# Liz490/multimodal_alzheimer

Hardware: AMD Instinct MI355X
Metric: volumes/sec fwd+bwd, 3D-ResNet-10 @128^3 bf16, 1/2/4/8 MI355X; % HBM roofline (higher is better)
Workload: dtype bf16; 1 GPU; BASELINE config 2: Anat_CNN ResNet-10 MRI-only, 1x128^3, batch 8/GPU, weighted CE, Adam, fwd+bwd+step; global_batch=8, parallelism=dp1, step_launch=hip graph replay

## Files before the change

### multimodal_alzheimer_amd/csrc/conv.hip

```cpp
#include <cstring>

#include "common.h"
#include "reduce.h"
#include "patchconv.h"
#include "pointwise.h"
#include "stem.h"

namespace {

constexpr int MAXTAPS = 344;
constexpr int TAPB = ((3 * MAXTAPS * 4 + 15) / 16) * 16;
constexpr int RB = 128;

struct Geom {
  int M, Nd, Cs, K, Kpad, cs_shift, taps, nb;
  int Ds, Hs, Ws, Dd, Hd, Wd;
  int KD, KH, KW;
  int sd, sh, sw, pd, ph, pw, dd, dh, dw;
  const void* res;
  int relu;
};

enum { FWD = 0, DGRAD = 1 };

// ... 1272 lines not shown
                                                          dst, stats, st);
      if (cfg == 5)
        return launch_igemm_bm<T, 256, MODE, 256, 2, 4, 4, 64>(g, m_max, classes, src, w, bias,
                                                              dst, stats, st);
      if (cfg == 6)
        return launch_igemm_bm<T, 256, MODE, 256, 2, 4, 3, 64>(g, m_max, classes, src, w, bias,
                                                              dst, stats, st);
    }
  }
  const bool small = igemm_bm(m_max * classes, g) == 64;
  if constexpr (sizeof(T) == 2) {
    if (igemm_nst(g, MODE) == 3) {
      if (bn_of(g) == 64)
        return small ? launch_igemm_bm<T, 64, MODE, 64, 2, 2, 3>(g, m_max, classes, src, w, bias, dst, stats, st)
                     : launch_igemm_bm<T, 64, MODE, 128, 2, 2, 3>(g, m_max, classes, src, w, bias, dst, stats, st);
      return small ? launch_igemm_bm<T, 128, MODE, 64, 2, 2, 3>(g, m_max, classes, src, w, bias, dst, stats, st)
                   : launch_igemm_bm<T, 128, MODE, 128, 2, 2, 3>(g, m_max, classes, src, w, bias, dst, stats, st);
    }
  }
  if (bn_of(g) == 64)
    return small ? launch_igemm_bm<T, 64, MODE, 64>(g, m_max, classes, src, w, bias, dst, stats, st)
                 : launch_igemm_bm<T, 64, MODE, 128>(g, m_max, classes, src, w, bias, dst, stats, st);
  return small ? launch_igemm_bm<T, 128, MODE, 64>(g, m_max, classes, src, w, bias, dst, stats, st)
               : launch_igemm_bm<T, 128, MODE, 128>(g, m_max, classes, src, w, bias, dst, stats, st);
}

template <int MODE>
int run_igemm(const Geom& g, int dtype, int64_t m_max, int classes, const void* src,
              const void* w, const float* bias, void* dst, float* stats, hipStream_t st) {
  if (dtype == MMAD_BF16)
    return run_igemm_t<u16, MODE>(g, m_max, classes, src, w, bias, dst, stats, st);
  return run_igemm_t<float, MODE>(g, m_max, classes, src, w, bias, dst, stats, st);
}

int wgrad_xcd() {
  static const int v = [] { const char* e = getenv("MMAD_WGRAD_XCD"); return e ? atoi(e) : 1; }();
  return v;
}

template <typename T, int BMW, int WBK, int NST, int WBNT, int WGM, int WGN, bool XFIX>
int launch_wgrad_x(const Geom& g, const WSplit& sp, const void* x, const void* dy, float* ws,
                   hipStream_t st) {
  const size_t lds = TAPB + NST * WBK * (BMW + WBNT) * sizeof(T);
  static const bool ok = set_lds(wgrad_kernel<T, BMW, WBK, NST, WBNT, WGM, WGN, XFIX>, lds);
  if (!ok) return MMAD_EUNSUPPORTED;
  const uint32_t xb = (uint32_t)((int64_t)g.nb * g.Ds * g.Hs * g.Ws * g.Cs * sizeof(T));
  const uint32_t yb = (uint32_t)((int64_t)g.M * g.Nd * sizeof(T));
  dim3 grid((unsigned)cdiv(g.K, WBNT), (unsigned)cdiv(g.Nd, BMW), (unsigned)sp.splits);
  hipLaunchKernelGGL((wgrad_kernel<T, BMW, WBK, NST, WBNT, WGM, WGN, XFIX>), grid,
                     dim3(64 * WGM * WGN), lds, st, g, (const T*)x, (const T*)dy, ws,
                     sp.m_per_split, xb, yb, wgrad_xcd());
  return launch_status();
}

template <typename T, int BMW, int WBK, int NST, int WBNT = WBN, int WGM = 2, int WGN = 2>
int launch_wgrad_k(const Geom& g, const WSplit& sp, const void* x, const void* dy, float* ws,
                   hipStream_t st) {
  if ((int64_t)g.nb * g.Ds * g.Hs * g.Ws * g.Cs * (int64_t)sizeof(T) >= (int64_t(1) << 31) ||
      (int64_t)g.M * g.Nd * (int64_t)sizeof(T) >= (int64_t(1) << 31))
    return MMAD_EUNSUPPORTED;
  if (WBK % g.Wd == 0)
    return launch_wgrad_x<T, BMW, WBK, NST, WBNT, WGM, WGN, true>(g, sp, x, dy, ws, st);
  return launch_wgrad_x<T, BMW, WBK, NST, WBNT, WGM, WGN, false>(g, sp, x, dy, ws, st);
}

int wgrad_1x1_nst() {
  static const int v = [] { const char* e = getenv("MMAD_WGRAD_1X1_NST"); return e ? atoi(e) : 3; }();
  return v;
}

template <typename T, int BMW>
int launch_wgrad(const Geom& g, const WSplit& sp, const void* x, const void* dy, float* ws,
                 hipStream_t st) {
  if (g.taps == 1 && wgrad_1x1_nst() == 3) return launch_wgrad_k<T, BMW, 32, 3>(g, sp, x, dy, ws, st);
  return launch_wgrad_k<T, BMW, 32, 2>(g, sp, x, dy, ws, st);
}

unsigned grid_for(int64_t total, int block = 256) {
  return (unsigned)std::max<int64_t>(1, std::min<int64_t>(cdiv(total, block), 65536));
}

enum Leaf { STEM, LATTICE5, LATTICE_ZP, LATTICE, LATTICE8, PATCHZ, PATCH, S2, PW, IGEMM, NONE };
enum Epi { EPI_NONE, EPI_RES, EPI_BNSUM };
bool leaf_has(Leaf l, Epi e) {
  if (e == EPI_RES) return l != STEM && l != PW;
  if (e == EPI_BNSUM) return l == LATTICE_ZP || l == LATTICE8 || l == PATCH;
  return true;
}
struct Route { Leaf leaf; int64_t tiles; };

Route resolve(const mmad_conv_desc* d, const Geom& g, int dtype, Epi epi, bool launch = true) {
  const Route none{NONE, -1};
  auto pick = [&](Leaf l, int64_t tiles) { return leaf_has(l, epi) ? Route{l, tiles} : none; };
  const bool u = d != nullptr && unfolded(d);
  if (u && epi != EPI_NONE) return none;
  if (u && mmad_stem::fwd_ok(d, dtype) && stem_kernel_on())
    return pick(STEM, mmad_stem::fwd_stats_rows(d));
  if (launch && !geom_ok(g, dtype)) return none;
  if (!u && dtype == MMAD_BF16) {
    const mmad_patch::Geo q = patch_geo(g);
    if (g.sd == 1 && g.sh == 1 && g.sw == 1) {
      if (mmad_lattice5::ok(q)) return pick(LATTICE5, mmad_lattice5::tiles(q));
      const bool zp = mmad_lattice_zp::ok(q);
      const int64_t lt = zp ? mmad_lattice_zp::tiles(q) : mmad_lattice::tiles(q);
      if (mmad_lattice::ok(q, lt)) return pick(zp ? LATTICE_ZP : LATTICE, lt);
      if (mmad_lattice8::ok(q)) return pick(LATTICE8, mmad_lattice8::tiles(q));
      if (mmad_patch::ok(q))
        return mmad_patchz::ok(q) ? pick(PATCHZ, mmad_patchz::tiles(q))
                                  : pick(PATCH, mmad_patch::tiles(q));
    }
    if (mmad_s2::ok(q, g.sd, g.sh, g.sw)) return pick(S2, mmad_s2::tiles(q));
  }
  if (d != nullptr && leaf_has(PW, epi) && mmad_pw::fwd_ok(d, dtype))
    return pick(PW, mmad_pw::fwd_tiles(d));
  return pick(IGEMM, cdiv(g.M, fwd_tile_rows(g, dtype)));
}

int launch_route(const Route& r, const mmad_conv_desc* d, const Geom& g, int dtype,
                 const mmad_patch::Geo& q, const void* x, const void* wp, const float* bias,
                 void* y, float* stats, void* stream) {
  switch (r.leaf) {
    case STEM: return mmad_stem::fwd(d, x, wp, bias, y, stats, stream);
    case LATTICE5: return mmad_lattice5::fwd(q, x, wp, bias, y, stats, stream);
    case LATTICE_ZP: return mmad_lattice_zp::fwd(q, x, wp, bias, y, stats, stream);
    case LATTICE: return mmad_lattice::fwd(q, x, wp, bias, y, stats, stream);
    case LATTICE8: return mmad_lattice8::fwd(q, x, wp, bias, y, stats, stream);
    case PATCHZ: return mmad_patchz::fwd(q, x, wp, bias, y, stats, stream);
    case PATCH: return mmad_patch::fwd(q, x, wp, bias, y, stats, stream);
    case S2: return mmad_s2::fwd(q, g.sd, g.sh, g.sw, x, wp, bias, y, stats, stream);
    case PW: return mmad_pw::fwd(d, x, wp, bias, y, stats, stream);
    case IGEMM: return run_igemm<FWD>(g, dtype, g.M, 1, x, wp, bias, y, stats, as_stream(stream));
    case NONE: break;
  }
  return MMAD_EUNSUPPORTED;
}

Route dgrad_fwd_route(const mmad_conv_desc* d, int dtype, Epi epi, Geom* gf) {
  if (!desc_ok(d) || (dtype != MMAD_F32 && dtype != MMAD_BF16) || unfolded(d) ||
      mmad_pw::ok(d, dtype) || !dgrad_as_fwd(d))
    return Route{NONE, -1};
  *gf = dgrad_fwd_geom(d, dtype);
  return resolve(nullptr, *gf, dtype, epi);
}

}

extern "C" {

int mmad_set_kernel_variant(const char* name, int value) {
  if (name == nullptr) return -1;
  if (std::strcmp(name, "lattice_zp") == 0) return mmad_lattice_zp::set_mode(value);
  if (std::strcmp(name, "lattice") == 0) return mmad_lattice::set_mode(value);
  if (std::strcmp(name, "lattice8") == 0) return mmad_lattice8::set_mode(value);
  if (std::strcmp(name, "lattice5") == 0) return mmad_lattice5::set_mode(value);
  if (std::strcmp(name, "pool_run") == 0) return mmad_pool::set_run_mode(value);
  if (std::strcmp(name, "patchz") == 0) return mmad_patchz::set_mode(value);
  if (std::strcmp(name, "pw_wg3_dedup") == 0) return mmad_pw::set_wg3_dedup(value);
  return -1;
}

int64_t mmad_conv_packed_elems(const mmad_conv_desc* d, int dtype, int for_dgrad) {
  if (!desc_ok(d)) return -1;
  const Geom g = for_dgrad ? dgrad_geom(d, dtype) : fwd_geom(d, dtype);
  return (int64_t)g.Nd * g.Kpad;
}

int mmad_conv_pack_weight_scaled(const mmad_conv_desc* d, int dtype, const float* w,
                                 const float* scale, void* wp, int for_dgrad, void* stream);

int mmad_conv_pack_weight(const mmad_conv_desc* d, int dtype, const float* w, void* wp,
                          int for_dgrad, void* stream) {
  return mmad_conv_pack_weight_scaled(d, dtype, w, nullptr, wp, for_dgrad, stream);
}

int mmad_conv_pack_weight_scaled(const mmad_conv_desc* d, int dtype, const float* w,
                                 const float* scale, void* wp, int for_dgrad, void* stream) {
  if (!desc_ok(d)) return MMAD_EBADSHAPE;
  if (dtype != MMAD_F32 && dtype != MMAD_BF16) return MMAD_EBADDTYPE;
  if (!w || !wp) return MMAD_ENULL;
  if (for_dgrad && unfolded(d)) return MMAD_EUNSUPPORTED;
  const Geom g = for_dgrad ? dgrad_geom(d, dtype) : fwd_geom(d, dtype);
  if (!geom_ok(g, dtype)) return MMAD_EUNSUPPORTED;
  const int mode = for_dgrad ? 1 : (unfolded(d) ? 2 : 0);
  const int flip = for_dgrad && dgrad_as_fwd(d);
  const int64_t total = (int64_t)g.Nd * g.Kpad;
  if (scale != nullptr && (mode != 0 || g.Kpad != g.K)) return MMAD_EUNSUPPORTED;
  if (mode != 2 && g.Kpad == g.K) {
    const int R = mode == 0 ? d->ci : d->co;
    const int Cc = mode == 0 ? g.taps : d->ci * g.taps;
    const int B = mode == 0 ? d->co : 1;
    const int64_t ob = mode == 0 ? g.Kpad : 0, oj1 = mode == 0 ? 0 : g.Kpad;
    const int jd = g.taps, oj2 = mode == 0 ? d->ci : d->co;
    dim3 grid((unsigned)cdiv(Cc, 64), (unsigned)cdiv(R, 64), (unsigned)B);
    if (dtype == MMAD_BF16)
      hipLaunchKernelGGL(pack_transpose_kernel<u16>, grid, dim3(256), 0, as_stream(stream), w,
                         (u16*)wp, R, Cc, ob, jd, oj1, oj2, flip, scale);
    else
      hipLaunchKernelGGL(pack_transpose_kernel<float>, grid, dim3(256), 0, as_stream(stream), w,
                         (float*)wp, R, Cc, ob, jd, oj1, oj2, flip, scale);
    return launch_status();
  }
  if (dtype == MMAD_BF16)
    hipLaunchKernelGGL(pack_weight_kernel<u16>, dim3(grid_for(total)), dim3(256), 0,
                       as_stream(stream), w, (u16*)wp, g.Nd, g.Kpad, g.K, g.Cs, g.cs_shift,
                       g.taps, mode, d->ci, d->kw, flip);
  else
    hipLaunchKernelGGL(pack_weight_kernel<float>, dim3(grid_for(total)), dim3(256), 0,
                       as_stream(stream), w, (float*)wp, g.Nd, g.Kpad, g.K, g.Cs, g.cs_shift,
                       g.taps, mode, d->ci, d->kw, flip);
  return launch_status();
}

int mmad_conv_pack_job(const mmad_conv_desc* d, int dtype, int for_dgrad, const float* w,
                       void* wp, int64_t tile0, mmad_pack_job* job) {
  if (!desc_ok(d)) return MMAD_EBADSHAPE;
  if (dtype != MMAD_F32 && dtype != MMAD_BF16) return MMAD_EBADDTYPE;
  if (!w || !wp || !job) return MMAD_ENULL;
  if (unfolded(d)) return MMAD_EUNSUPPORTED;
  const Geom g = for_dgrad ? dgrad_geom(d, dtype) : fwd_geom(d, dtype);
  if (!geom_ok(g, dtype) || g.Kpad != g.K) return MMAD_EUNSUPPORTED;
  const bool fw = !for_dgrad;
  mmad_pack_job j{};
  j.w = w;
  j.w_packed = wp;
  j.rows = fw ? d->co * d->ci : d->co;
  j.rdiv = fw ? d->ci : d->co;
  j.cols = fw ? g.taps : d->ci * g.taps;
  j.batch = 1;
  j.jdiv = g.taps;
  j.ostride_j2 = fw ? d->ci : d->co;
  j.ostride_b = fw ? g.Kpad : 0;
  j.ostride_j1 = fw ? 0 : g.Kpad;
  const bool narrow = j.cols <= 32;
  j.tiles_x = (int)cdiv(j.cols, narrow ? 32 : 64);
  j.tiles_y = (int)cdiv(j.rows, narrow ? 128 : 64);
  j.pad_ = for_dgrad && dgrad_as_fwd(d);
  j.tile0 = tile0;
  *job = j;
  return MMAD_OK;
}

int mmad_conv_pack_dual_job(const mmad_conv_desc* d, int dtype, const float* w, void* w_fwd,
                            void* w_dgrad, int64_t tile0, mmad_pack_dual* job) {
  if (!desc_ok(d)) return MMAD_EBADSHAPE;
  if (dtype != MMAD_BF16) return MMAD_EUNSUPPORTED;
  if (!w || !w_fwd || !w_dgrad || !job) return MMAD_ENULL;
  if (unfolded(d)) return MMAD_EUNSUPPORTED;
  const Geom gf = fwd_geom(d, dtype), gd = dgrad_geom(d, dtype);
  if (!geom_ok(gf, dtype) || !geom_ok(gd, dtype) || gf.Kpad != gf.K || gd.Kpad != gd.K)
    return MMAD_EUNSUPPORTED;
  if (d->ci % 16 || d->co % 16 || gf.taps > 27) return MMAD_EUNSUPPORTED;
  mmad_pack_dual j{};
  j.w = w;
  j.w_fwd = w_fwd;
  j.w_dgrad = w_dgrad;
  j.co = d->co;
  j.ci = d->ci;
  j.taps = gf.taps;
  j.flip = dgrad_as_fwd(d) ? 1 : 0;
  j.tile0 = tile0;
  *job = j;
  return MMAD_OK;
}

int64_t mmad_pack_dual_tiles(const mmad_pack_dual* job) {
  return job ? (int64_t)(job->co / 16) * (job->ci / 16) : -1;
}

int mmad_conv_pack_dual_batch(int dtype, int njobs, const mmad_pack_dual* jobs,
                              int64_t total_tiles, void* stream) {
  if (njobs <= 0 || total_tiles <= 0 || total_tiles > INT32_MAX) return MMAD_EBADSHAPE;
  if (!jobs) return MMAD_ENULL;
  if (dtype != MMAD_BF16) return MMAD_EBADDTYPE;
  hipLaunchKernelGGL(pack_dual_kernel, dim3((unsigned)total_tiles), dim3(256), 0,
                     as_stream(stream), jobs, njobs);
  return launch_status();
}

int64_t mmad_pack_job_tiles(const mmad_pack_job* job) {
  return job ? (int64_t)job->tiles_x * job->tiles_y * job->batch : -1;
}

int mmad_conv_pack_batch(int dtype, int njobs, const mmad_pack_job* jobs, int64_t total_tiles,
                         void* stream) {
  if (njobs <= 0 || total_tiles <= 0 || total_tiles > INT32_MAX) return MMAD_EBADSHAPE;
  if (!jobs) return MMAD_ENULL;
  if (dtype == MMAD_BF16)
    hipLaunchKernelGGL(pack_batch_kernel<u16>, dim3((unsigned)total_tiles), dim3(256), 0,
                       as_stream(stream), jobs, njobs);
  else if (dtype == MMAD_F32)
    hipLaunchKernelGGL(pack_batch_kernel<float>, dim3((unsigned)total_tiles), dim3(256), 0,
                       as_stream(stream), jobs, njobs);
  else
    return MMAD_EBADDTYPE;
  return launch_status();
}

int64_t mmad_conv_unfolded_elems(const mmad_conv_desc* d) {
  if (!desc_ok(d) || !unfolded(d)) return -1;
  return (int64_t)d->n * d->di * d->hi * d->wo * 8;
}

int mmad_conv_unfold_input(const mmad_conv_desc* d, int in_dtype, const void* x, int dtype,
                           void* xu, void* stream) {
  if (!desc_ok(d) || !unfolded(d)) return MMAD_EBADSHAPE;
  if (d->kw > 8) return MMAD_EUNSUPPORTED;
// ... 377 lines not shown
```

### multimodal_alzheimer_amd/csrc/lattice8.hip

```cpp
#include <atomic>
#include <cstdlib>
#include <type_traits>

#include "bnsum.h"
#include "common.h"
#include "patchconv.h"

namespace {

constexpr int S8 = 8;
constexpr int NC = 8;
constexpr int PL8 = S8 * S8 * NC;
constexpr int RB8 = 64;
constexpr int KC8 = RB8 / 2;
constexpr int PLANE8 = PL8 * RB8;
constexpr int BN8 = 64;
constexpr int BTAP8 = BN8 * RB8;
constexpr int TPS8 = 9;
constexpr int BSLOT8 = TPS8 * BTAP8;
constexpr int NSL8 = 2;
constexpr int NPL8 = 2;
constexpr int RING8 = NPL8 * PLANE8;
constexpr int ZERO8 = RING8 + NSL8 * BSLOT8;
constexpr int MAIN8 = ZERO8 + RB8;
constexpr int CROW8 = BN8 * 2 + 16;
constexpr int EPI8 = PL8 * CROW8 + 7 * 2 * BN8 * 4;
constexpr int LDS8 = MAIN8 > EPI8 ? MAIN8 : EPI8;
constexpr int NT8 = 512;

struct L8 {
  int nb, Cs, Nd, Kpad, nbn, nchunk;
  const u16* res;
  int relu;
  int D, H, W, nz;
  const u16* bny;
  const float *bnsc, *bnsh, *bnmu, *bnis;
  float* bnparts;
};

__device__ __forceinline__ int swz8(int row) { return 3 * ((row >> 3) & 1); }

template <int TN, int NFR>
struct Fr8 {
  bf16x8 b[TN];
  bf16x8 a[NFR];
};

template <int WM, int KY, int WR>
__device__ constexpr bool row_ok(int f) {
  return WR * WM + (f >> 2) + KY >= 0 && WR * WM + (f >> 2) + KY < S8;
}

template <int TN, int WM, int KY, int KX, int WR>
__device__ __forceinline__ void read8(const char* bsl, const char* pl, const uint32_t (&ao)[2],
                                      const char* zp, bool lhi, Fr8<TN, 4 * WR>& f) {
#pragma unroll
  for (int j = 0; j < TN; ++j)
    f.b[j] = *reinterpret_cast<const bf16x8*>(bsl + (KX + 1) * BTAP8 + j * 16 * RB8);
#pragma unroll
  for (int q = 0; q < 4 * WR; ++q) {
    if (row_ok<WM, KY, WR>(q)) {
      constexpr int dummy = 0;
      const int ty = WR * WM + (q >> 2) + KY + dummy, x0 = 2 * (q & 3) + KX;
      const int base = (ty * S8 + x0) * NC * RB8;
      const char* p = pl + base + ao[KX & 1];
      if (KX == -1 && (q & 3) == 0) p = lhi ? p : zp;
      if (KX == 1 && (q & 3) == 3) p = lhi ? zp : p;
      f.a[q] = *reinterpret_cast<const bf16x8*>(p);
    }
  }
}

template <int TN, int WM, int KY, int WR>
__device__ __forceinline__ void mma8(f32x4 (&acc)[4 * WR][TN], const Fr8<TN, 4 * WR>& f) {
#pragma unroll
  for (int q = 0; q < 4 * WR; ++q)
    if (row_ok<WM, KY, WR>(q)) {
#pragma unroll
      for (int j = 0; j < TN; ++j)
        acc[q][j] = __builtin_amdgcn_mfma_f32_16x16x32_bf16(f.a[q], f.b[j], acc[q][j], 0, 0, 0);
    }
}

template <int TN, int WM, int KY, int WR>
__device__ __forceinline__ void stage8(f32x4 (&acc)[4 * WR][TN], const char* bsl,
                                       const char* pl, const uint32_t (&ao)[2], const char* zp,
                                       bool lhi) {
  Fr8<TN, 4 * WR> f0, f1;
  read8<TN, WM, KY, -1, WR>(bsl, pl, ao, zp, lhi, f0);
  read8<TN, WM, KY, 0, WR>(bsl, pl, ao, zp, lhi, f1);
  mma8<TN, WM, KY, WR>(acc, f0);
  read8<TN, WM, KY, 1, WR>(bsl, pl, ao, zp, lhi, f0);
  mma8<TN, WM, KY, WR>(acc, f1);
  mma8<TN, WM, KY, WR>(acc, f0);
}

template <int TN, bool RAG, int WR>
__global__ __launch_bounds__(NT8) void lattice8_conv_kernel(L8 g, const u16* __restrict__ src,
                                                            const u16* __restrict__ wgt,
                                                            const float* __restrict__ bias,
                                                            u16* __restrict__ dst,
                                                            float* __restrict__ stats) {
  extern __shared__ __attribute__((aligned(16))) char smem[];
  char* ring = smem + RING8;
  const int tid = threadIdx.x, lane = tid & 63;
  const int wave = __builtin_amdgcn_readfirstlane(tid >> 6);
  const int nwg = gridDim.x, bid = blockIdx.x;
  const int xcd = bid & 7, qq = nwg >> 3, rr = nwg & 7;
  const int tile = (xcd < rr ? xcd * (qq + 1) : rr * (qq + 1) + (xcd - rr) * qq) + (bid >> 3);
  const int nt = tile % g.nbn;
  const int t2 = tile / g.nbn;
  const int NZ = RAG ? g.nz : S8;
  const int tz = t2 % NZ, n = t2 / NZ;
  constexpr int NFR = 4 * WR;
  constexpr int NWM = 8 / WR, NWN = WR;
  constexpr int BW = 16 * TN * NWN;
  const int n0 = nt * BW;
  constexpr int E = 2 * S8;

  if (tid < RB8 / 16)
    *reinterpret_cast<u32x4*>(smem + ZERO8 + tid * 16) = u32x4{0u, 0u, 0u, 0u};

  const int lrow = lane >> 2;
  int rzk[4];
  uint32_t pofs[4];
#pragma unroll
  for (int k = 0; k < 4; ++k) {
    const int row = (wave * 4 + k) * 16 + lrow;
    const int pos = row >> 3, c = row & 7;
    const int ty = pos >> 3, tx = pos & 7;
    const int pch = (lane & 3) ^ swz8(row);
    if constexpr (RAG) {
      const int y = ((c >> 1) & 1) + 2 * ty, x = (c & 1) + 2 * tx;
      pofs[k] = (uint32_t)((((c >> 2) * g.H + y) * g.W + x) * g.Cs + pch * 8) * 2u;
      rzk[k] = (y < g.H && x < g.W) ? (c >> 2) : -(1 << 20);
    } else {
      const int v = ((c >> 2) * E + ((c >> 1) & 1) + 2 * ty) * E + (c & 1) + 2 * tx;
      pofs[k] = (uint32_t)(v * g.Cs + pch * 8) * 2u;
      rzk[k] = 0;
    }
  }
  const int64_t svox = RAG ? (int64_t)g.D * g.H * g.W : (int64_t)E * E * E;
  const __amdgpu_buffer_rsrc_t rsx = __builtin_amdgcn_make_buffer_rsrc(
      (void*)(src + (int64_t)n * svox * g.Cs), 0,
      (int)__builtin_amdgcn_readfirstlane((uint32_t)(svox * g.Cs * 2)), 0x00020000);
  auto issue_plane_at = [&](int p, int zr, int cc) {
    char* pb = smem + p * PLANE8;
    if constexpr (RAG) {
      constexpr uint32_t OOB = 0x80000000u;
      const int zp = 2 * (tz - 1 + zr);
      const uint32_t zoff = (uint32_t)(zp * g.H * g.W * g.Cs + cc * KC8) * 2u;
#pragma unroll
      for (int k = 0; k < 4; ++k) {
        const bool ok = rzk[k] >= 0 && rzk[k] + zp >= 0 && rzk[k] + zp < g.D;
        buf_lds16_asm(ok ? pofs[k] + zoff : OOB, rsx, lds_addr_of(pb + (wave * 4 + k) * 1024));
      }
    } else {
      const uint32_t zoff = (uint32_t)(2 * (tz - 1 + zr) * E * E * g.Cs + cc * KC8) * 2u;
#pragma unroll
      for (int k = 0; k < 4; ++k) {
        uint32_t o = pofs[k];
        asm volatile("" : "+v"(o));
        buf_lds16_asm(o + zoff, rsx, lds_addr_of(pb + (wave * 4 + k) * 1024));
      }
    }
  };
  constexpr int QB = BW / 16;
  constexpr int NQ9 = 9 * BW / 16, WI9 = (NQ9 + 7) / 8;
  const __amdgpu_buffer_rsrc_t rsw = __builtin_amdgcn_make_buffer_rsrc(
      (void*)wgt, 0, (int)__builtin_amdgcn_readfirstlane((uint32_t)(g.Nd * g.Kpad * 2)),
      0x00020000);
  uint32_t wofs9[WI9];
#pragma unroll
  for (int h = 0; h < WI9; ++h) {
    const int q = min(wave + 8 * h, NQ9 - 1);
    const int row = (q % QB) * 16 + lrow;
    wofs9[h] = (uint32_t)((n0 + row) * g.Kpad + ((lane & 3) ^ swz8(row)) * 8 + (q / QB) * g.Cs) *
               2u;
  }
  auto issue_b9 = [&](int cc, int t0, int sl) {
    const uint32_t so = (uint32_t)(t0 * g.Cs + cc * KC8) * 2u;
#pragma unroll
    for (int h = 0; h < WI9; ++h) {
      const int q = min(wave + 8 * h, NQ9 - 1);
      uint32_t o = wofs9[h];
      asm volatile("" : "+v"(o));
      buf_lds16_asm(o + so, rsw, lds_addr_of(ring + sl * BSLOT8 + (q / QB) * BTAP8 + (q % QB) * 1024));
    }
  };
  const int kz0 = tz == 0 ? 0 : -1, kz1 = tz == NZ - 1 ? 0 : 1;
  const int nkz = kz1 - kz0 + 1;
  const int wm = wave % NWM, wn = wave / NWM;
  const int lr = lane & 15, lk = lane >> 4;
  const bool lhi = (lr >> 3) != 0;
  uint32_t ao[2];
  ao[0] = lr * RB8 + ((lk ^ swz8(lr)) << 4);
  ao[1] = lr * RB8 + ((lk ^ (3 - swz8(lr))) << 4);
  const char* zp = smem + ZERO8 + (lk << 4);
  const uint32_t b_lane = (wn * 16 * TN + lr) * RB8 + ((lk ^ swz8(lr)) << 4);
  f32x4 acc[NFR][TN];
#pragma unroll
  for (int i = 0; i < NFR; ++i)
#pragma unroll
    for (int j = 0; j < TN; ++j) acc[i][j] = f32x4{0.f, 0.f, 0.f, 0.f};

  auto run9 = [&](auto wmc) {
    constexpr int WM = decltype(wmc)::value;
    const int n9 = g.nchunk * nkz;
    issue_plane_at(0, kz0 + 1, 0);
    issue_b9(0, (kz0 + 1) * 9, 0);
    int e = 0;
    for (int c = 0; c < g.nchunk; ++c)
      for (int kzi = 0; kzi < nkz; ++kzi, ++e) {
        wait_vm_lgkm0<0>();
        raw_barrier();
        if (e + 1 < n9) {
          const int c1 = kzi + 1 < nkz ? c : c + 1, kz1 = kz0 + (kzi + 1 < nkz ? kzi + 1 : 0);
          issue_plane_at((e + 1) & 1, kz1 + 1, c1);
          issue_b9(c1, (kz1 + 1) * 9, (e + 1) & 1);
        }
        const char* pl = smem + (e & 1) * PLANE8;
        const char* bs = ring + (e & 1) * BSLOT8 + b_lane;
        stage8<TN, WM, -1, WR>(acc, bs, pl, ao, zp, lhi);
        stage8<TN, WM, 0, WR>(acc, bs + 3 * BTAP8, pl, ao, zp, lhi);
        stage8<TN, WM, 1, WR>(acc, bs + 6 * BTAP8, pl, ao, zp, lhi);
      }
  };
  auto dispatch = [&](auto wmc) {
    if constexpr (decltype(wmc)::value < NWM) run9(wmc);
  };
  switch (wm) {
    case 0: dispatch(std::integral_constant<int, 0>{}); break;
    case 1: dispatch(std::integral_constant<int, 1>{}); break;
    case 2: dispatch(std::integral_constant<int, 2>{}); break;
    case 3: dispatch(std::integral_constant<int, 3>{}); break;
    case 4: dispatch(std::integral_constant<int, 4>{}); break;
    case 5: dispatch(std::integral_constant<int, 5>{}); break;
    case 6: dispatch(std::integral_constant<int, 6>{}); break;
    default: dispatch(std::integral_constant<int, 7>{}); break;
  }
  __syncthreads();

  auto dst_vox = [&](int row) -> int64_t {
    const int pos = row >> 3, c = row & 7;
    const int ty = pos >> 3, tx = pos & 7;
    if constexpr (RAG) {
      const int z = (c >> 2) + 2 * tz, y = ((c >> 1) & 1) + 2 * ty, x = (c & 1) + 2 * tx;
      if (z >= g.D || y >= g.H || x >= g.W) return -1;
      return (((int64_t)n * g.D + z) * g.H + y) * g.W + x;
    }
    return (((int64_t)n * E + (c >> 2) + 2 * tz) * E + ((c >> 1) & 1) + 2 * ty) * E + (c & 1) +
           2 * tx;
  };
  u16* ctile = reinterpret_cast<u16*>(smem);
  uint32_t vmask = 0xffffffffu;
  if constexpr (RAG) {
    vmask = 0;
#pragma unroll 1
    for (int b = 0; b < 4 * NFR; ++b) {
      const int q = b >> 2, e = b & 3;
      const int row = ((WR * wm + (q >> 2)) * S8 + 2 * (q & 3)) * NC + lk * 4 + e;
      if (dst_vox(row) >= 0) vmask |= 1u << b;
    }
  }
  float cs[TN], cq[TN];
#pragma unroll
  for (int j = 0; j < TN; ++j) {
    cs[j] = 0.f;
    cq[j] = 0.f;
    const int col = wn * 16 * TN + j * 16 + lr;
    const float bv = bias != nullptr ? bias[n0 + col] : 0.f;
#pragma unroll
    for (int q = 0; q < NFR; ++q) {
      const int ty = WR * wm + (q >> 2);
#pragma unroll
      for (int e = 0; e < 4; ++e) {
        const int row = (ty * S8 + 2 * (q & 3)) * NC + lk * 4 + e;
        const float v = acc[q][j][e] + bv;
        ctile[row * (CROW8 / 2) + col] = f2bf(v);
        if ((vmask >> (q * 4 + e)) & 1u) {
          cs[j] += v;
          cq[j] += v * v;
        }
      }
    }
  }
  __syncthreads();
  constexpr int CPR = BW / 8;
  static_assert(NT8 % CPR == 0, "a thread keeps one channel vector in the store loop");
  if (g.bny != nullptr) {
    BnSum bs;
    bs.init(g.bnsc, g.bnsh, g.bnmu, g.bnis, n0 + (tid % CPR) * 8);
#pragma unroll
    for (int hh = 0; hh < PL8 * CPR / NT8; ++hh) {
      const int qd = tid + NT8 * hh;
      const int row = qd / CPR, c8 = qd % CPR;
      const int64_t dv = dst_vox(row);
      if (RAG && dv < 0) continue;
      const int64_t o = dv * g.Nd + n0 + c8 * 8;
      const u32x4 v = *reinterpret_cast<const u32x4*>(reinterpret_cast<const char*>(ctile) +
                                                      row * CROW8 + c8 * 16);
      const u32x4 yv = *reinterpret_cast<const u32x4*>(g.bny + o);
      *reinterpret_cast<u32x4*>(dst + o) = v;
      bs.add(v, yv);
    }
    __syncthreads();
    bnsum_flush(bs, reinterpret_cast<float*>(smem), CPR, NT8, g.bnparts, n * NZ + tz, g.Nd, n0);
    return;
  }
#pragma unroll
  for (int hh = 0; hh < PL8 * CPR / NT8; ++hh) {
    const int qd = tid + NT8 * hh;
    const int row = qd / CPR, c8 = qd % CPR;
    const int64_t dv = dst_vox(row);
    if (RAG && dv < 0) continue;
    const int64_t o = dv * g.Nd + n0 + c8 * 8;
    u32x4 v = *reinterpret_cast<const u32x4*>(reinterpret_cast<const char*>(ctile) +
                                              row * CROW8 + c8 * 16);
    if (g.res != nullptr || g.relu) v = epi_res_relu(v, g.res ? g.res + o : nullptr, g.relu);
    *reinterpret_cast<u32x4*>(dst + o) = v;
  }
  if (stats != nullptr) {
    float* red = reinterpret_cast<float*>(smem + PL8 * CROW8);
#pragma unroll
    for (int j = 0; j < TN; ++j) {
      cs[j] += __shfl_xor(cs[j], 16, 64);
      cs[j] += __shfl_xor(cs[j], 32, 64);
      cq[j] += __shfl_xor(cq[j], 16, 64);
      cq[j] += __shfl_xor(cq[j], 32, 64);
    }
    if (wm > 0 && lk == 0) {
#pragma unroll
      for (int j = 0; j < TN; ++j) {
        const int col = wn * 16 * TN + j * 16 + lr;
        red[(wm - 1) * 2 * BW + col] = cs[j];
        red[(wm - 1) * 2 * BW + BW + col] = cq[j];
      }
    }
    __syncthreads();
    if (wm == 0 && lk == 0) {
      const int mt = n * NZ + tz;
#pragma unroll
      for (int j = 0; j < TN; ++j) {
        const int col = wn * 16 * TN + j * 16 + lr;
        float ss = cs[j], qs = cq[j];
        for (int w = 1; w < NWM; ++w) {
          ss += red[(w - 1) * 2 * BW + col];
          qs += red[(w - 1) * 2 * BW + BW + col];
        }
        stats[((int64_t)mt * 2) * g.Nd + n0 + col] = ss;
        stats[((int64_t)mt * 2 + 1) * g.Nd + n0 + col] = qs;
      }
    }
  }
}

std::atomic<int> g_lattice8_mode{-1};
int lattice8_mode() {
  int v = g_lattice8_mode.load(std::memory_order_relaxed);
  if (v < 0) {
    const char* e = getenv("MMAD_LATTICE8");
    int expect = -1;
    g_lattice8_mode.compare_exchange_strong(expect, e ? atoi(e) : 1);
    v = g_lattice8_mode.load(std::memory_order_relaxed);
  }
  return v;
}

int l8_rows() {
  static const int v = [] {
    const char* e = getenv("MMAD_L8_ROWS");
    return e && atoi(e) == 2 ? 2 : 1;
  }();
  return v;
}

}

namespace mmad_lattice8 {

int set_mode(int v) {
  const int prev = lattice8_mode();
  if (v >= 0) g_lattice8_mode.store(v, std::memory_order_relaxed);
  return prev;
}

static bool exact8(const mmad_patch::Geo& q) {
  constexpr int E = 2 * S8;
  return q.Ds == E && q.Hs == E && q.Ws == E && q.Dd == E && q.Hd == E && q.Wd == E;
}
static bool ragged8(const mmad_patch::Geo& q) {
  static const int mode = [] {
    const char* e = getenv("MMAD_LATTICE_RAGGED");
    return e ? atoi(e) : 1;
  }();
  return mode > 0 && !exact8(q) && q.Ds == q.Dd && q.Hs == q.Hd && q.Ws == q.Wd &&
         (q.Hs + 1) / 2 <= S8 && (q.Ws + 1) / 2 <= S8 &&
         (int64_t)q.Ds * q.Hs * q.Ws * q.Cs * 2 < (int64_t(1) << 31);
}
static int planes8(const mmad_patch::Geo& q) { return exact8(q) ? S8 : (q.Ds + 1) / 2; }

bool ok(const mmad_patch::Geo& q) {
  if (lattice8_mode() <= 0) return false;
  if (q.KD != 3 || q.KH != 3 || q.KW != 3) return false;
  if (q.dd != 2 || q.dh != 2 || q.dw != 2 || q.pd != 2 || q.ph != 2 || q.pw != 2) return false;
  if (!exact8(q) && !ragged8(q)) return false;
  if (q.Cs % KC8 || q.Nd % 32 || q.Kpad != 27 * q.Cs) return false;
  if (lattice8_mode() == 1 && (int64_t)q.nb * planes8(q) * (q.Nd / 32) < 256) return false;
  return (int64_t)q.Ds * q.Hs * q.Ws * q.Cs * 2 < (int64_t(1) << 31) &&
         (int64_t)q.Nd * q.Kpad * 2 < (int64_t(1) << 31);
}

int64_t tiles(const mmad_patch::Geo& q) { return (int64_t)q.nb * planes8(q); }

int fwd(const mmad_patch::Geo& q, const void* src, const void* wp, const float* bias,
        void* dst, float* stats, void* stream) {
  if (!mmad_lattice8::ok(q)) return MMAD_EUNSUPPORTED;
  auto attr1 = [](const void* k) {
    return hipFuncSetAttribute(k, hipFuncAttributeMaxDynamicSharedMemorySize, LDS8) ==
           hipSuccess;
  };
  static const bool attr =
      attr1((const void*)lattice8_conv_kernel<2, false, 2>) &&
      attr1((const void*)lattice8_conv_kernel<1, false, 2>) &&
      attr1((const void*)lattice8_conv_kernel<2, true, 2>) &&
      attr1((const void*)lattice8_conv_kernel<1, true, 2>) &&
      attr1((const void*)lattice8_conv_kernel<4, false, 1>) &&
      attr1((const void*)lattice8_conv_kernel<2, false, 1>) &&
      attr1((const void*)lattice8_conv_kernel<4, true, 1>) &&
      attr1((const void*)lattice8_conv_kernel<2, true, 1>);
  if (!attr) return MMAD_EUNSUPPORTED;
  const bool rag = !exact8(q);
  const int nz = planes8(q);
  const bool wide = q.Nd % BN8 == 0 && (int64_t)q.nb * nz * (q.Nd / BN8) >= 256;
  L8 g{};
  g.nb = q.nb; g.Cs = q.Cs; g.Nd = q.Nd; g.Kpad = q.Kpad;
  g.nbn = q.Nd / (wide ? BN8 : 32);
  g.nchunk = q.Cs / KC8;
  g.res = reinterpret_cast<const u16*>(q.res);
  g.relu = q.relu;
  g.D = q.Ds; g.H = q.Hs; g.W = q.Ws; g.nz = nz;
  g.bny = reinterpret_cast<const u16*>(q.bny);
  g.bnsc = q.bnsc; g.bnsh = q.bnsh; g.bnmu = q.bnmu; g.bnis = q.bnis;
  g.bnparts = q.bnparts;
  if (g.bny != nullptr && (stats != nullptr || g.res != nullptr || g.relu || bias != nullptr))
    return MMAD_EUNSUPPORTED;
  const int64_t nblk = (int64_t)q.nb * nz * g.nbn;
  auto go = [&](auto kern) {
    hipLaunchKernelGGL(kern, dim3((unsigned)nblk), dim3(NT8), LDS8, as_stream(stream), g,
                       (const u16*)src, (const u16*)wp, bias, (u16*)dst, stats);
  };
  if (l8_rows() == 1) {
    if (wide) rag ? go(lattice8_conv_kernel<4, true, 1>) : go(lattice8_conv_kernel<4, false, 1>);
    else rag ? go(lattice8_conv_kernel<2, true, 1>) : go(lattice8_conv_kernel<2, false, 1>);
  } else {
    if (wide) rag ? go(lattice8_conv_kernel<2, true, 2>) : go(lattice8_conv_kernel<2, false, 2>);
    else rag ? go(lattice8_conv_kernel<1, true, 2>) : go(lattice8_conv_kernel<1, false, 2>);
  }
  return launch_status();
}

}
```

### multimodal_alzheimer_amd/csrc/patchconv.h

```cpp
#pragma once
#include <stdint.h>

#include "../../include/mmad.h"

namespace mmad_patch {
struct Geo {
  int nb, Cs, Nd, Kpad;
  int Ds, Hs, Ws, Dd, Hd, Wd;
  int KD, KH, KW, pd, ph, pw, dd, dh, dw;
  const void* res = nullptr;
  int relu = 0;
  const void* bny = nullptr;
  const float* bnsc = nullptr;
  const float* bnsh = nullptr;
  const float* bnmu = nullptr;
  const float* bnis = nullptr;
  float* bnparts = nullptr;
};
bool ok(const Geo& g);
int64_t tiles(const Geo& g);
int fwd(const Geo& g, const void* src, const void* wp, const float* bias, void* dst,
        float* stats, void* stream);
}

namespace mmad_patchz {
int set_mode(int v);
bool ok(const mmad_patch::Geo& g);
int64_t tiles(const mmad_patch::Geo& g);
int fwd(const mmad_patch::Geo& g, const void* src, const void* wp, const float* bias, void* dst,
        float* stats, void* stream);
}

namespace mmad_lattice {
int set_mode(int v);
bool ok(const mmad_patch::Geo& g, int64_t fill_tiles);
int64_t tiles(const mmad_patch::Geo& g);
int fwd(const mmad_patch::Geo& g, const void* src, const void* wp, const float* bias, void* dst,
        float* stats, void* stream);
bool wgrad_ok(const mmad_patch::Geo& g);
int64_t wgrad_workspace(const mmad_patch::Geo& g);
int wgrad(const mmad_patch::Geo& g, const void* x, const void* dy, float* ws, int* splits,
          void* stream);
}

namespace mmad_s2 {
bool ok(const mmad_patch::Geo& g, int sd, int sh, int sw);
int64_t tiles(const mmad_patch::Geo& g);
int fwd(const mmad_patch::Geo& g, int sd, int sh, int sw, const void* src, const void* wp,
        const float* bias, void* dst, float* stats, void* stream);
bool dgrad_ok(const mmad_conv_desc* d);
int dgrad(const mmad_conv_desc* d, const void* dy, const void* wpt, void* dx, void* stream);
}

namespace mmad_lattice_zp {
int set_mode(int v);
bool ok(const mmad_patch::Geo& g);
int64_t tiles(const mmad_patch::Geo& g);
int fwd(const mmad_patch::Geo& g, const void* src, const void* wp, const float* bias, void* dst,
        float* stats, void* stream);
}

namespace mmad_lattice5 {
int set_mode(int v);
bool ok(const mmad_patch::Geo& g);
int64_t tiles(const mmad_patch::Geo& g);
int fwd(const mmad_patch::Geo& g, const void* src, const void* wp, const float* bias, void* dst,
        float* stats, void* stream);
bool wgrad_ok(const mmad_patch::Geo& g);
int64_t wgrad_workspace(const mmad_patch::Geo& g);
int wgrad(const mmad_patch::Geo& g, const void* x, const void* dy, float* ws, int* splits,
          void* stream);
}

namespace mmad_lattice8 {
int set_mode(int v);
bool ok(const mmad_patch::Geo& g);
int64_t tiles(const mmad_patch::Geo& g);
int fwd(const mmad_patch::Geo& g, const void* src, const void* wp, const float* bias, void* dst,
        float* stats, void* stream);
}

namespace mmad_pwgrad {
bool ok(const mmad_patch::Geo& g);
int64_t workspace(const mmad_patch::Geo& g);
int wgrad(const mmad_patch::Geo& g, const void* x, const void* dy, float* ws, int* splits,
          void* stream);
}

namespace mmad_pool {
int set_run_mode(int v);
}
```

Baseline: 2797 volumes/sec.

## Add x-walk lattice8 conv variant that reuses A fragments across KX taps

Adds an x-walk form of the lattice8 3x3x3 conv kernel for the exact (non-ragged) grid. Each wave now owns a full 8-wide row of positions with a 4x2 wave split, so a row of A fragments loaded once from LDS serves all three KX taps, cutting LDS reads per MFMA. LDS reads are interleaved with MFMAs through sched_group_barrier, and the swizzle, zero padding and BN stats reduction are reworked to match. The variant is on by default and replaces the old MMAD_L8_ROWS=2 path. It adds register pressure (8xTN accumulators) and a more complex epilogue.

```diff
diff --git a/multimodal_alzheimer_amd/csrc/conv.hip b/multimodal_alzheimer_amd/csrc/conv.hip
--- a/multimodal_alzheimer_amd/csrc/conv.hip
+++ b/multimodal_alzheimer_amd/csrc/conv.hip
@@ -1448,6 +1448,7 @@
   if (std::strcmp(name, "lattice_zp") == 0) return mmad_lattice_zp::set_mode(value);
   if (std::strcmp(name, "lattice") == 0) return mmad_lattice::set_mode(value);
   if (std::strcmp(name, "lattice8") == 0) return mmad_lattice8::set_mode(value);
+  if (std::strcmp(name, "lattice8_xwalk") == 0) return mmad_lattice8::set_xwalk(value);
   if (std::strcmp(name, "lattice5") == 0) return mmad_lattice5::set_mode(value);
   if (std::strcmp(name, "pool_run") == 0) return mmad_pool::set_run_mode(value);
   if (std::strcmp(name, "patchz") == 0) return mmad_patchz::set_mode(value);
diff --git a/multimodal_alzheimer_amd/csrc/lattice8.hip b/multimodal_alzheimer_amd/csrc/lattice8.hip
--- a/multimodal_alzheimer_amd/csrc/lattice8.hip
+++ b/multimodal_alzheimer_amd/csrc/lattice8.hip
@@ -1,6 +1,7 @@
 #include <atomic>
 #include <cstdlib>
 #include <type_traits>
+#include <utility>
 
 #include "bnsum.h"
 #include "common.h"
@@ -22,7 +23,7 @@
 constexpr int NPL8 = 2;
 constexpr int RING8 = NPL8 * PLANE8;
 constexpr int ZERO8 = RING8 + NSL8 * BSLOT8;
-constexpr int MAIN8 = ZERO8 + RB8;
+constexpr int MAIN8 = ZERO8 + NC * RB8;
 constexpr int CROW8 = BN8 * 2 + 16;
 constexpr int EPI8 = PL8 * CROW8 + 7 * 2 * BN8 * 4;
 constexpr int LDS8 = MAIN8 > EPI8 ? MAIN8 : EPI8;
@@ -39,63 +40,135 @@
 };
 
 __device__ __forceinline__ int swz8(int row) { return 3 * ((row >> 3) & 1); }
-
-template <int TN, int NFR>
+__device__ __forceinline__ int swz8x(int row) { return 3 * (((row >> 3) ^ (row >> 6)) & 1); }
+
+template <int TN>
 struct Fr8 {
   bf16x8 b[TN];
-  bf16x8 a[NFR];
+  bf16x8 a[4];
 };
 
-template <int WM, int KY, int WR>
-__device__ constexpr bool row_ok(int f) {
-  return WR * WM + (f >> 2) + KY >= 0 && WR * WM + (f >> 2) + KY < S8;
-}
-
-template <int TN, int WM, int KY, int KX, int WR>
+template <int WM, int KY>
+__device__ constexpr bool row_ok() {
+  return WM + KY >= 0 && WM + KY < S8;
+}
+
+template <int TN, int WM, int KY, int KX>
 __device__ __forceinline__ void read8(const char* bsl, const char* pl, const uint32_t (&ao)[2],
-                                      const char* zp, bool lhi, Fr8<TN, 4 * WR>& f) {
+                                      const char* zp, bool lhi, Fr8<TN>& f) {
 #pragma unroll
   for (int j = 0; j < TN; ++j)
     f.b[j] = *reinterpret_cast<const bf16x8*>(bsl + (KX + 1) * BTAP8 + j * 16 * RB8);
 #pragma unroll
-  for (int q = 0; q < 4 * WR; ++q) {
-    if (row_ok<WM, KY, WR>(q)) {
-      constexpr int dummy = 0;
-      const int ty = WR * WM + (q >> 2) + KY + dummy, x0 = 2 * (q & 3) + KX;
+  for (int q = 0; q < 4; ++q) {
+    if (row_ok<WM, KY>()) {
+      const int ty = WM + KY, x0 = 2 * q + KX;
       const int base = (ty * S8 + x0) * NC * RB8;
       const char* p = pl + base + ao[KX & 1];
-      if (KX == -1 && (q & 3) == 0) p = lhi ? p : zp;
-      if (KX == 1 && (q & 3) == 3) p = lhi ? zp : p;
+      if (KX == -1 && q == 0) p = lhi ? p : zp;
+      if (KX == 1 && q == 3) p = lhi ? zp : p;
       f.a[q] = *reinterpret_cast<const bf16x8*>(p);
     }
   }
 }
 
-template <int TN, int WM, int KY, int WR>
-__device__ __forceinline__ void mma8(f32x4 (&acc)[4 * WR][TN], const Fr8<TN, 4 * WR>& f) {
-#pragma unroll
-  for (int q = 0; q < 4 * WR; ++q)
-    if (row_ok<WM, KY, WR>(q)) {
+template <int TN, int WM, int KY>
+__device__ __forceinline__ void mma8(f32x4 (&acc)[4][TN], const Fr8<TN>& f) {
+#pragma unroll
+  for (int q = 0; q < 4; ++q)
+    if (row_ok<WM, KY>()) {
 #pragma unroll
       for (int j = 0; j < TN; ++j)
         acc[q][j] = __builtin_amdgcn_mfma_f32_16x16x32_bf16(f.a[q], f.b[j], acc[q][j], 0, 0, 0);
     }
 }
 
-template <int TN, int WM, int KY, int WR>
-__device__ __forceinline__ void stage8(f32x4 (&acc)[4 * WR][TN], const char* bsl,
-                                       const char* pl, const uint32_t (&ao)[2], const char* zp,
-                                       bool lhi) {
-  Fr8<TN, 4 * WR> f0, f1;
-  read8<TN, WM, KY, -1, WR>(bsl, pl, ao, zp, lhi, f0);
-  read8<TN, WM, KY, 0, WR>(bsl, pl, ao, zp, lhi, f1);
-  mma8<TN, WM, KY, WR>(acc, f0);
-  read8<TN, WM, KY, 1, WR>(bsl, pl, ao, zp, lhi, f0);
-  mma8<TN, WM, KY, WR>(acc, f1);
-  mma8<TN, WM, KY, WR>(acc, f0);
-}
-
-template <int TN, bool RAG, int WR>
+template <int TN, int WM, int KY>
+__device__ __forceinline__ void stage8(f32x4 (&acc)[4][TN], const char* bsl, const char* pl,
+                                       const uint32_t (&ao)[2], const char* zp, bool lhi) {
+  Fr8<TN> f0, f1;
+  read8<TN, WM, KY, -1>(bsl, pl, ao, zp, lhi, f0);
+  read8<TN, WM, KY, 0>(bsl, pl, ao, zp, lhi, f1);
+  mma8<TN, WM, KY>(acc, f0);
+  read8<TN, WM, KY, 1>(bsl, pl, ao, zp, lhi, f0);
+  mma8<TN, WM, KY>(acc, f1);
+  mma8<TN, WM, KY>(acc, f0);
+}
+
+template <int WP, int KY, int X0, int X1>
+__device__ __forceinline__ void read_ax(const char* pl, const uint32_t (&ao)[2],
+                                        const char* const (&zl)[2], bool lhi,
+                                        bf16x8 (&a)[S8]) {
+#pragma unroll
+  for (int x = X0; x < X1; ++x) {
+    const int k = (x + KY + 2) & 1;
+    const char* p = pl + ((2 * WP + KY) * S8 + x) * NC * RB8 + ao[k];
+    if (WP == 0 && KY == -1) p = lhi ? p : zl[k];
+    if (WP == 3 && KY == 1) p = lhi ? zl[k] : p;
+    a[x] = *reinterpret_cast<const bf16x8*>(p);
+  }
+}
+
+template <int TN>
+__device__ __forceinline__ void read_bx(const char* bsl, int tap, bf16x8 (&b)[TN]) {
+#pragma unroll
+  for (int j = 0; j < TN; ++j)
+    b[j] = *reinterpret_cast<const bf16x8*>(bsl + tap * BTAP8 + j * 16 * RB8);
+}
+
+template <int TN, int WP>
+__device__ __forceinline__ void stage8x(f32x4 (&acc)[S8][TN], const char* bsl, const char* pl,
+                                        const uint32_t (&ao)[2], const char* const (&zl)[2],
+                                        bool lhi) {
+  bf16x8 a[2][S8], b[3][TN];
+  read_bx<TN>(bsl, 0, b[0]);
+  read_ax<WP, -1, 0, S8>(pl, ao, zl, lhi, a[0]);
+  read_bx<TN>(bsl, 1, b[1]);
+  __builtin_amdgcn_sched_barrier(0);
+  auto tap = [&](auto tc) __attribute__((always_inline)) {
+    constexpr int T = decltype(tc)::value, R = T / 3, KX = T % 3 - 1;
+    constexpr int X0 = 3 * (KX + 1), X1 = KX == 1 ? S8 : X0 + 3;
+    constexpr int NR = (T + 2 < TPS8 ? TN : 0) + (R < 2 ? X1 - X0 : 0);
+    constexpr int NM = (KX == 0 ? S8 : S8 - 1) * TN;
+    static_assert(NM >= NR, "a read per MFMA gap");
+    if constexpr (T + 2 < TPS8) read_bx<TN>(bsl, T + 2, b[(T + 2) % 3]);
+    if constexpr (R < 2) read_ax<WP, R, X0, X1>(pl, ao, zl, lhi, a[(R + 1) & 1]);
+#pragma unroll
+    for (int x = 0; x < S8; ++x)
+      if (x + KX >= 0 && x + KX < S8) {
+#pragma unroll
+        for (int j = 0; j < TN; ++j)
+          acc[x][j] = __builtin_amdgcn_mfma_f32_16x16x32_bf16(a[R & 1][x + KX], b[T % 3][j],
+                                                              acc[x][j], 0, 0, 0);
+      }
+#ifndef L8X_NO_INTERLEAVE
+#pragma unroll
+    for (int k = 0; k < NR; ++k) {
+      __builtin_amdgcn_sched_group_barrier(0x008, 1, 0);
+      __builtin_amdgcn_sched_group_barrier(0x100, 1, 0);
+    }
+    if constexpr (NM > NR) __builtin_amdgcn_sched_group_barrier(0x008, NM - NR, 0);
+#endif
+  };
+  [&]<int... T>(std::integer_sequence<int, T...>) {
+    (tap(std::integral_constant<int, T>{}), ...);
+  }(std::make_integer_sequence<int, TPS8>{});
+}
+
+__device__ __forceinline__ float sqsum16(const float (&v)[16], bool fused) {
+#pragma clang fp contract(off)
+  float qf = __builtin_fmaf(v[0], v[0], v[1] * v[1]);
+  float qu = v[0] * v[0];
+  qu = qu + v[1] * v[1];
+#pragma unroll
+  for (int i = 2; i < 16; ++i) {
+    qf = __builtin_fmaf(v[i], v[i], qf);
+    qu = qu + v[i] * v[i];
+  }
+  return fused ? qf : qu;
+}
+
+template <int TN, bool RAG, bool XW = false>
 __global__ __launch_bounds__(NT8) void lattice8_conv_kernel(L8 g, const u16* __restrict__ src,
                                                             const u16* __restrict__ wgt,
                                                             const float* __restrict__ bias,
@@ -112,13 +185,14 @@
   const int t2 = tile / g.nbn;
   const int NZ = RAG ? g.nz : S8;
   const int tz = t2 % NZ, n = t2 / NZ;
-  constexpr int NFR = 4 * WR;
-  constexpr int NWM = 8 / WR, NWN = WR;
+  static_assert(!XW || !RAG, "the x-walk form is the exact grid's");
+  constexpr int NFR = XW ? S8 : 4;
+  constexpr int NWM = XW ? 4 : 8, NWN = XW ? 2 : 1;
   constexpr int BW = 16 * TN * NWN;
   const int n0 = nt * BW;
   constexpr int E = 2 * S8;
 
-  if (tid < RB8 / 16)
+  if (tid < (XW ? NC : 1) * RB8 / 16)
     *reinterpret_cast<u32x4*>(smem + ZERO8 + tid * 16) = u32x4{0u, 0u, 0u, 0u};
 
   const int lrow = lane >> 2;
@@ -129,7 +203,7 @@
     const int row = (wave * 4 + k) * 16 + lrow;
     const int pos = row >> 3, c = row & 7;
     const int ty = pos >> 3, tx = pos & 7;
-    const int pch = (lane & 3) ^ swz8(row);
+    const int pch = (lane & 3) ^ (XW ? swz8x(row) : swz8(row));
     if constexpr (RAG) {
       const int y = ((c >> 1) & 1) + 2 * ty, x = (c & 1) + 2 * tx;
       pofs[k] = (uint32_t)((((c >> 2) * g.H + y) * g.W + x) * g.Cs + pch * 8) * 2u;
@@ -197,6 +271,15 @@
   ao[0] = lr * RB8 + ((lk ^ swz8(lr)) << 4);
   ao[1] = lr * RB8 + ((lk ^ (3 - swz8(lr))) << 4);
   const char* zp = smem + ZERO8 + (lk << 4);
+  const char* zl[2] = {zp, zp};
+  if constexpr (XW) {
+#pragma unroll
+    for (int k = 0; k < 2; ++k) {
+      const uint32_t o = (lr & 7) * RB8 + ((lk ^ (3 * (k ^ (int)lhi))) << 4);
+      ao[k] = (lhi ? S8 * NC * RB8 : 0) + o;
+      zl[k] = smem + ZERO8 + o;
+    }
+  }
   const uint32_t b_lane = (wn * 16 * TN + lr) * RB8 + ((lk ^ swz8(lr)) << 4);
   f32x4 acc[NFR][TN];
 #pragma unroll
@@ -221,9 +304,13 @@
         }
         const char* pl = smem + (e & 1) * PLANE8;
         const char* bs = ring + (e & 1) * BSLOT8 + b_lane;
-        stage8<TN, WM, -1, WR>(acc, bs, pl, ao, zp, lhi);
-        stage8<TN, WM, 0, WR>(acc, bs + 3 * BTAP8, pl, ao, zp, lhi);
-        stage8<TN, WM, 1, WR>(acc, bs + 6 * BTAP8, pl, ao, zp, lhi);
+        if constexpr (XW) {
+          stage8x<TN, WM>(acc, bs, pl, ao, zl, lhi);
+        } else {
+          stage8<TN, WM, -1>(acc, bs, pl, ao, zp, lhi);
+          stage8<TN, WM, 0>(acc, bs + 3 * BTAP8, pl, ao, zp, lhi);
+          stage8<TN, WM, 1>(acc, bs + 6 * BTAP8, pl, ao, zp, lhi);
+        }
       }
   };
   auto dispatch = [&](auto wmc) {
@@ -259,23 +346,43 @@
 #pragma unroll 1
     for (int b = 0; b < 4 * NFR; ++b) {
       const int q = b >> 2, e = b & 3;
-      const int row = ((WR * wm + (q >> 2)) * S8 + 2 * (q & 3)) * NC + lk * 4 + e;
+      const int row = (wm * S8 + 2 * q) * NC + lk * 4 + e;
       if (dst_vox(row) >= 0) vmask |= 1u << b;
     }
   }
-  float cs[TN], cq[TN];
+  float cs[TN], cq[TN], cso[TN], cqo[TN];
 #pragma unroll
   for (int j = 0; j < TN; ++j) {
     cs[j] = 0.f;
     cq[j] = 0.f;
+    cso[j] = 0.f;
+    cqo[j] = 0.f;
     const int col = wn * 16 * TN + j * 16 + lr;
     const float bv = bias != nullptr ? bias[n0 + col] : 0.f;
+    if constexpr (XW) {
+      float ve[16], vo[16];
+#pragma unroll
+      for (int x = 0; x < S8; ++x) {
+#pragma unroll
+        for (int e = 0; e < 4; ++e) {
+          const int row = ((2 * wm + (lk >> 1)) * S8 + x) * NC + (lk & 1) * 4 + e;
+          const float v = acc[x][j][e] + bv;
+          ctile[row * (CROW8 / 2) + col] = f2bf(v);
+          (x & 1 ? vo : ve)[(x >> 1) * 4 + e] = v;
+          if (x & 1) cso[j] += v;
+          else cs[j] += v;
+        }
+      }
+      const bool fused = wn * TN + j != 2 * TN - 1;
+      cq[j] = sqsum16(ve, fused);
+      cqo[j] = sqsum16(vo, fused);
+      continue;
+    }
 #pragma unroll
     for (int q = 0; q < NFR; ++q) {
-      const int ty = WR * wm + (q >> 2);
 #pragma unroll
       for (int e = 0; e < 4; ++e) {
-        const int row = (ty * S8 + 2 * (q & 3)) * NC + lk * 4 + e;
+        const int row = (wm * S8 + 2 * q) * NC + lk * 4 + e;
         const float v = acc[q][j][e] + bv;
         ctile[row * (CROW8 / 2) + col] = f2bf(v);
         if ((vmask >> (q * 4 + e)) & 1u) {
@@ -322,6 +429,39 @@
   }
   if (stats != nullptr) {
     float* red = reinterpret_cast<float*>(smem + PL8 * CROW8);
+    if constexpr (XW) {
+      const int ty = 2 * wm + (lk >> 1);
+#pragma unroll
+      for (int j = 0; j < TN; ++j) {
+        cs[j] += __shfl_xor(cs[j], 16, 64);
+        cso[j] += __shfl_xor(cso[j], 16, 64);
+        cs[j] += cso[j];
+        cq[j] += __shfl_xor(cq[j], 16, 64);
+        cqo[j] += __shfl_xor(cqo[j], 16, 64);
+        cq[j] += cqo[j];
+        const int col = wn * 16 * TN + j * 16 + lr;
+        if (ty > 0 && (lk & 1) == 0) {
+          red[(ty - 1) * 2 * BW + col] = cs[j];
+          red[(ty - 1) * 2 * BW + BW + col] = cq[j];
+        }
+      }
+      __syncthreads();
+      if (wm == 0 && lk == 0) {
+        const int mt = n * NZ + tz;
+#pragma unroll
+        for (int j = 0; j < TN; ++j) {
+          const int col = wn * 16 * TN + j * 16 + lr;
+          float ss = cs[j], qs = cq[j];
+          for (int w = 1; w < S8; ++w) {
+            ss += red[(w - 1) * 2 * BW + col];
+            qs += red[(w - 1) * 2 * BW + BW + col];
+          }
+          stats[((int64_t)mt * 2) * g.Nd + n0 + col] = ss;
+          stats[((int64_t)mt * 2 + 1) * g.Nd + n0 + col] = qs;
+        }
+      }
+      return;
+    }
 #pragma unroll
     for (int j = 0; j < TN; ++j) {
       cs[j] += __shfl_xor(cs[j], 16, 64);
@@ -367,11 +507,15 @@
   return v;
 }
 
-int l8_rows() {
-  static const int v = [] {
-    const char* e = getenv("MMAD_L8_ROWS");
-    return e && atoi(e) == 2 ? 2 : 1;
-  }();
+std::atomic<int> g_l8_xwalk{-1};
+int l8_xwalk() {
+  int v = g_l8_xwalk.load(std::memory_order_relaxed);
+  if (v < 0) {
+    const char* e = getenv("MMAD_L8_XWALK");
+    int expect = -1;
+    g_l8_xwalk.compare_exchange_strong(expect, e ? (atoi(e) != 0) : 1);
+    v = g_l8_xwalk.load(std::memory_order_relaxed);
+  }
   return v;
 }
 
@@ -382,6 +526,12 @@
 int set_mode(int v) {
   const int prev = lattice8_mode();
   if (v >= 0) g_lattice8_mode.store(v, std::memory_order_relaxed);
+  return prev;
+}
+
+int set_xwalk(int v) {
+  const int prev = l8_xwalk();
+  if (v >= 0) g_l8_xwalk.store(v != 0, std::memory_order_relaxed);
   return prev;
 }
 
@@ -421,14 +571,12 @@
            hipSuccess;
   };
   static const bool attr =
-      attr1((const void*)lattice8_conv_kernel<2, false, 2>) &&
-      attr1((const void*)lattice8_conv_kernel<1, false, 2>) &&
-      attr1((const void*)lattice8_conv_kernel<2, true, 2>) &&
-      attr1((const void*)lattice8_conv_kernel<1, true, 2>) &&
-      attr1((const void*)lattice8_conv_kernel<4, false, 1>) &&
-      attr1((const void*)lattice8_conv_kernel<2, false, 1>) &&
-      attr1((const void*)lattice8_conv_kernel<4, true, 1>) &&
-      attr1((const void*)lattice8_conv_kernel<2, true, 1>);
+      attr1((const void*)lattice8_conv_kernel<4, false>) &&
+      attr1((const void*)lattice8_conv_kernel<2, false>) &&
+      attr1((const void*)lattice8_conv_kernel<4, true>) &&
+      attr1((const void*)lattice8_conv_kernel<2, true>) &&
+      attr1((const void*)lattice8_conv_kernel<2, false, true>) &&
+      attr1((const void*)lattice8_conv_kernel<1, false, true>);
   if (!attr) return MMAD_EUNSUPPORTED;
   const bool rag = !exact8(q);
   const int nz = planes8(q);
@@ -450,12 +598,11 @@
     hipLaunchKernelGGL(kern, dim3((unsigned)nblk), dim3(NT8), LDS8, as_stream(stream), g,
                        (const u16*)src, (const u16*)wp, bias, (u16*)dst, stats);
   };
-  if (l8_rows() == 1) {
-    if (wide) rag ? go(lattice8_conv_kernel<4, true, 1>) : go(lattice8_conv_kernel<4, false, 1>);
-    else rag ? go(lattice8_conv_kernel<2, true, 1>) : go(lattice8_conv_kernel<2, false, 1>);
+  if (!rag && l8_xwalk()) {
+    wide ? go(lattice8_conv_kernel<2, false, true>) : go(lattice8_conv_kernel<1, false, true>);
   } else {
-    if (wide) rag ? go(lattice8_conv_kernel<2, true, 2>) : go(lattice8_conv_kernel<2, false, 2>);
-    else rag ? go(lattice8_conv_kernel<1, true, 2>) : go(lattice8_conv_kernel<1, false, 2>);
+    if (wide) rag ? go(lattice8_conv_kernel<4, true>) : go(lattice8_conv_kernel<4, false>);
+    else rag ? go(lattice8_conv_kernel<2, true>) : go(lattice8_conv_kernel<2, false>);
   }
   return launch_status();
 }
diff --git a/multimodal_alzheimer_amd/csrc/patchconv.h b/multimodal_alzheimer_amd/csrc/patchconv.h
--- a/multimodal_alzheimer_amd/csrc/patchconv.h
+++ b/multimodal_alzheimer_amd/csrc/patchconv.h
@@ -74,6 +74,7 @@
 
 namespace mmad_lattice8 {
 int set_mode(int v);
+int set_xwalk(int v);
 bool ok(const mmad_patch::Geo& g);
 int64_t tiles(const mmad_patch::Geo& g);
 int fwd(const mmad_patch::Geo& g, const void* src, const void* wp, const float* bias, void* dst,
```

After: 2826 volumes/sec, median of 6. +1.0%, better.
